# dyfcalid/CameraCalibration

Measured on AMD Instinct MI355X. Metric: stitched BEV frames/sec (4-cam 1280x960->1080x1080), higher is better.
Workload: dtype u8

## Files before the change

cameracalibration_amd/csrc/bevw_unit.h:

```cpp
#pragma once
#include <algorithm>
#include <cstring>
#include <vector>

#ifndef BEVW_UNIT_STORE16
#define BEVW_UNIT_STORE16 0
#endif

namespace bevw {

constexpr int kUnitWaves = 4;
constexpr int kUnitThreads = kUnitWaves * 64;
constexpr int kUnitMaxNQ = 4;
constexpr int kUnitMaxGR = 4;
constexpr int kUnitMaxGroups = kUnitMaxGR * kUnitThreads;
constexpr int kUnitMaxWidth = 256;
constexpr int kUnitClasses = 8;
constexpr int kUnitClassNQ[kUnitClasses] = {4, 4, 2, 1, 2, 1, 1, 4};
constexpr int kUnitClassGR[kUnitClasses] = {1, 2, 4, 4, 1, 4, 1, 4};
constexpr int kUnitClassCON[kUnitClasses] = {1, 1, 1, 1, 2, 2, 2, 1};
constexpr int kUnitClassBig = 7;
constexpr uint32_t kUnitSkip = 1u << 22;

struct UnitDesc {
// ... 19 lines not shown
    return k | (slot0 << 2) | (slot1 << 12) | ((code & 1023u) << 22);
}
__host__ __device__ __forceinline__ void unit_decode(uint32_t e, uint32_t &i0, uint32_t &i1, uint32_t &wxa, uint32_t &wy)
{
    const uint32_t fx = (e >> 22) & 31u, fy = e >> 27;
    i0 = e & 0xfffu;
    i1 = ((e >> 10) & 0xffcu) | (e & 3u);
    wxa = (i0 >> 2) != (i1 >> 2) ? ((32u - fx) | (fx << 8)) : 0u;
    wy = ((32u - fy) << 6) | (fy << 22);
}

constexpr uint32_t kUnitFracBits = 21;
__host__ __device__ __forceinline__ void unit_decode_wide(uint32_t e, uint32_t f, uint32_t &i0, uint32_t &i1, float &fx, float &fy)
{
    i0 = e & 0xfffu;
    i1 = ((e >> 10) & 0xffcu) | (e & 3u);
    fx = (float)((((e >> 22) & 31u) << 16) | (f & 0xffffu)) * (1.0f / (float)(1u << kUnitFracBits));
    fy = (float)(((e >> 27) << 16) | (f >> 16)) * (1.0f / (float)(1u << kUnitFracBits));
}
__host__ __device__ __forceinline__ void unit_repack16(int q, const uint32_t d[3], const uint32_t n[3], uint32_t o[4])
{
    o[0] = q == 0 ? d[0] : (q == 1 ? d[1] : d[2]);
    o[1] = q == 0 ? d[1] : (q == 1 ? d[2] : n[0]);
    o[2] = q == 0 ? d[2] : (q == 1 ? n[0] : n[1]);
    o[3] = q == 0 ? n[0] : (q == 1 ? n[1] : n[2]);
}
__host__ __device__ __forceinline__ bool unit_no_contributor(uint32_t e) { return ((e >> 2) & 1023u) == ((e >> 12) & 1023u); }
__host__ __device__ __forceinline__ uint32_t bilinear_pairs_f32(uint2 q0, uint2 q1, float fx, float fy)
{
    auto lerp = [](float a, float b, float t) { return fmaf(t, b - a, a); };
    auto ch = [&](uint32_t w0, uint32_t w1, int s) {
        const float t = lerp((float)((w0 >> s) & 255u), (float)((w0 >> (s + 8)) & 255u), fx);
        const float b = lerp((float)((w1 >> s) & 255u), (float)((w1 >> (s + 8)) & 255u), fx);
        return (uint32_t)rintf(lerp(t, b, fy));
    };
    return ch(q0.x, q1.x, 0) | (ch(q0.x, q1.x, 16) << 8) | (ch(q0.y, q1.y, 0) << 16);
}

static inline std::vector<uint32_t> unit_host_headers(const std::vector<int16_t> lut1[4], const std::vector<uint8_t> mask[4], int ncams, int fw, int fh,
                                                      int bw, int bh, int tiles_x, int tiles_y);

struct UnitPlanHost {
    std::vector<UnitDesc> desc;
    std::vector<uint32_t> entries;
    std::vector<uint32_t> gsrc;
    std::vector<uint32_t> list[kUnitClasses];
    std::vector<uint32_t> all;
    size_t claimed_tiles = 0;
    uint32_t skew = 0;
    bool wide = false;
    size_t lines = 0, sectors = 0;
    size_t cls_lines[kUnitClasses] = {}, cls_sectors[kUnitClasses] = {}, cls_pixels[kUnitClasses] = {}, cls_groups[kUnitClasses] = {};
};

struct UnitTuning {
    int max_groups = kUnitMaxGroups;
    int root_w = 256, root_h = 64;
    int min_w = 16;
    int line_cost = 2, sector_cost = 3;
    int align_lines = 1;
    int own_empty = 1;
    int own_double = 1;
    int wide_double = 1;
    int skew = 0;
    int row_order = 0;
    int own_padding = 1;
    int run_cost = 0;
    int stagger = 0;
    int big_class = 1;
};

static inline void unit_compile(const std::vector<int16_t> lut1[4], const std::vector<uint16_t> lut2[4], const std::vector<uint8_t> mask[4],
                                int ncams, int fw, int fh, int bw, int bh, int pitch, int tiles_x, int tiles_y, std::vector<uint32_t> &hdr,
                                UnitPlanHost &out, const UnitTuning &tune = UnitTuning(), const std::vector<uint32_t> *frac = nullptr)
{
    const bool wide = frac != nullptr;
    out.wide = wide;
    const uint32_t frame_bytes = (uint32_t)fw * fh * 3, gpr = (uint32_t)fw / 4;
    const size_t set_bytes = (size_t)frame_bytes * ncams;
    constexpr uint32_t kNone = 0xffffffffu;
    std::vector<uint8_t> own((size_t)tiles_x * tiles_y, 0);
    for (size_t t = 0; t < own.size(); ++t) {
        own[t] = (hdr[t] & (kHdrSlow | kHdrBlock)) ? 0 : ((hdr[t] & kHdrSecond) ? (tune.own_double ? 2 : 0) : 1);
        if ((hdr[t] & kHdrEmpty) && !tune.own_empty) own[t] = 0;
    }
    std::vector<uint32_t> poff[2], pcode[2], pfrac[2];
    std::vector<uint8_t> pmask[2];
    for (int k = 0; k < 2; ++k) {
        poff[k].assign((size_t)pitch * bh, kNone); pcode[k].assign((size_t)pitch * bh, 0u); pmask[k].assign((size_t)pitch * bh, 0);
        if (wide) pfrac[k].assign((size_t)pitch * bh, 0u);
    }
    for (int y = 0; y < bh; ++y)
        for (int x = 0; x < bw; ++x) {
            const size_t t = (size_t)(y / 8) * tiles_x + x / 32;
            if (!own[t]) continue;
            const size_t o = (size_t)y * bw + x;
            int count = 0;
            for (int c = 0; c < ncams; ++c) {
                const uint32_t m = mask[c][o];
                if (m == 0) continue;
                const int sx = lut1[c][o * 2], sy = lut1[c][o * 2 + 1];
                if (sx >= fw || sx + 1 < 0 || sy >= fh || sy + 1 < 0) continue;
                const uint32_t off = (uint32_t)c * frame_bytes + ((uint32_t)sy * fw + sx) * 3;
                if ((size_t)(off / 12u + gpr) * 12u + 16u > set_bytes || count >= 2) { own[t] = 0; break; }
                if (m != 255u && own[t] == 1) own[t] = tune.own_double ? 2 : 0;
                poff[count][(size_t)y * pitch + x] = off;
                if (wide) {
                    const uint32_t fx = frac[c][o * 2] & ((1u << kUnitFracBits) - 1u), fy = frac[c][o * 2 + 1] & ((1u << kUnitFracBits) - 1u);
                    pcode[count][(size_t)y * pitch + x] = (fx >> 16) | ((fy >> 16) << 5);
                    pfrac[count][(size_t)y * pitch + x] = (fx & 0xffffu) | (fy << 16);
                } else {
                    pcode[count][(size_t)y * pitch + x] = lut2[c][o] & (kQTab2 - 1);
                }
                pmask[count][(size_t)y * pitch + x] = (uint8_t)m;
                ++count;
            }
        }
    for (int y = 0; y < bh; ++y)
        for (int x = 0; x < bw; ++x)
            if (own[(size_t)(y / 8) * tiles_x + x / 32] == 0) poff[0][(size_t)y * pitch + x] = poff[1][(size_t)y * pitch + x] = kNone;
    int pass = 1;
    const int bw_own = tune.own_padding ? std::min(pitch, tiles_x * 32) : bw;
    auto owned = [&](int x, int y) { return x < bw_own && y < bh && own[(size_t)(y / 8) * tiles_x + x / 32] == pass; };
    const uint32_t P = (uint32_t)pitch * 3u;
    uint32_t skew = 0;
    int col_step = 16;
    if ((tune.skew == 64 || tune.skew == 32) && ((size_t)P * bh) % (size_t)tune.skew == 0) {
        const uint32_t m = (uint32_t)tune.skew / 4u, inv = tune.skew == 64 ? 11u : 3u;
        const uint32_t c = (m - ((P / 4u) * inv) % m) % m;
        if (c != 0) { skew = c | ((m - 1u) << 8); col_step = tune.skew; }
        else col_step = tune.skew;
    }
    out.skew = skew;
    const int min_w = std::max(col_step, tune.min_w);
    auto px_x = [&](int u, int y) { return u + unit_skew(skew, y); };

    std::vector<uint32_t> gstamp(set_bytes / 12 + 2, 0u), lstamp(set_bytes / 128 + 2, 0u);
    uint32_t stamp = 0;
    struct Stats { int groups, lines, pixels, quads; };
    auto cell_stats = [&](int x0, int y0, int w, int h) {
        Stats s = {0, 0, 0, 0};
        ++stamp;
        for (int y = y0; y < y0 + h; ++y)
            for (int u = x0; u < x0 + w; ++u) {
                const int x = px_x(u, y);
                if (x < 0 || x >= pitch) continue;
                if (!owned(x & ~3, y)) continue;
                if ((x & 3) == 0) ++s.quads;
                for (int con = 0; con < 2; ++con) {
                    const uint32_t off = poff[con][(size_t)y * pitch + x];
                    if (off == kNone) continue;
                    ++s.pixels;
                    for (uint32_t r = 0; r < 2; ++r) {
                        const uint32_t k = off / 12u + r * gpr;
                        if (gstamp[k] == stamp) continue;
                        gstamp[k] = stamp;
                        ++s.groups;
                        const uint32_t a = k * 12u;
                        for (uint32_t l = a >> 7; l <= (a + 15u) >> 7; ++l)
                            if (lstamp[l] != stamp) { lstamp[l] = stamp; ++s.lines; }
                    }
                }
            }
        return s;
    };
    auto write_sectors = [&](int x0, int y0, int w, int h) {
        long n = 0;
        for (int y = y0; y < y0 + h; ++y) {
            const int xa = std::max(0, px_x(x0, y)), xb = std::min(pitch, px_x(x0 + w, y));
            int run0 = -1;
            for (int x = xa; x <= xb; x += 4) {
                const bool in = x < xb && owned(x, y);
                if (in && run0 < 0) run0 = x;
                if (!in && run0 >= 0) {
                    const long a0 = ((long)y * pitch + run0) * 3, a1 = ((long)y * pitch + x) * 3;
                    n += (a1 - 1) / 64 - a0 / 64 + 1;
                    run0 = -1;
                }
            }
        }
        return n;
    };
    auto shrink = [&](int &x0, int &y0, int &w, int &h) {
        int ya = y0 + h, yb = y0, ua = x0 + w, ub = x0;
        for (int y = y0; y < y0 + h; ++y)
            for (int u = x0; u < x0 + w; u += 4) {
                const int x = px_x(u, y);
                if (x < 0 || x >= pitch || !owned(x, y)) continue;
                ya = std::min(ya, y); yb = std::max(yb, y + 1); ua = std::min(ua, u); ub = std::max(ub, u + 4);
            }
        if (yb <= ya) return;
        const int xa = x0 + (ua - x0) / col_step * col_step, xb = std::min(x0 + w, x0 + (ub - x0 + col_step - 1) / col_step * col_step);
        x0 = xa; w = xb - xa; y0 = ya; h = yb - ya;
    };
    auto lanes_log2 = [](int w) { int lq = 2; while ((4 << lq) < w) ++lq; return lq; };
    auto slots_needed = [&](int w, int h) { const int rps = 64 >> lanes_log2(w); return (h + rps - 1) / rps; };

    const int root_w = std::min(tune.root_w, kUnitMaxWidth);
    struct Order { uint64_t key; uint32_t entry; uint32_t row; uint64_t cost; };
    auto row_start = [&](int y0) {
        int xs = skew ? -col_step : 0;
        if (tune.stagger > 0) xs -= (((y0 / tune.root_h) * tune.stagger) % root_w) / col_step * col_step;
        return xs;
    };
    std::vector<Order> order;
    std::vector<uint32_t> keys, slot;
    auto emit = [&](int x0, int y0, int w, int h, const Stats &st) {
        keys.clear();
        for (int y = y0; y < y0 + h; ++y)
            for (int u = x0; u < x0 + w; ++u) {
                const int x = px_x(u, y);
                if (x < 0 || x >= pitch || !owned(x & ~3, y)) continue;
                for (int con = 0; con < 2; ++con) {
                    const uint32_t off = poff[con][(size_t)y * pitch + x];
                    if (off == kNone) continue;
                    keys.push_back(off / 12u);
                    keys.push_back(off / 12u + gpr);
                }
            }
        std::sort(keys.begin(), keys.end());
        keys.erase(std::unique(keys.begin(), keys.end()), keys.end());
        const int count = (int)keys.size();
        slot.assign((size_t)count, 0u);
        uint32_t used = 0;
        for (int i = 0; i < count;) {
            int j = i;
            while (j < count && (keys[(size_t)j] * 12u) >> 7 == (keys[(size_t)i] * 12u) >> 7) ++j;
            if (tune.align_lines && (used & 63u) + (uint32_t)(j - i) > 64u) used = (used + 63u) & ~63u;
            for (; i < j; ++i) slot[(size_t)i] = used++;
        }
        const int lq = lanes_log2(w), slots = slots_needed(w, h);
        int cls = -1, best = 1 << 30;
        for (int c = 0; c < kUnitClasses; ++c) {
            if (kUnitClassCON[c] != pass || kUnitClassNQ[c] * kUnitWaves < slots || kUnitClassGR[c] * kUnitThreads < (int)used + (wide ? 1 : 0)) continue;
            if (c == 4 && !tune.wide_double) continue;
            if (c == kUnitClassBig && !tune.big_class) continue;
            const int cost = kUnitClassNQ[c] * 64 + kUnitClassGR[c] * 14;
            if (cost < best) { best = cost; cls = c; }
        }
        if (cls < 0) return false;
        const int NQ = kUnitClassNQ[cls], GR = kUnitClassGR[cls], fpart = pass == 2 ? 3 : 1, parts = fpart + (wide ? pass : 0);
        const uint32_t zent = wide ? unit_entry(used, used, 0u, 0u) : 0u;
        UnitDesc d;
        d.pos = (uint32_t)(uint16_t)(int16_t)x0 | ((uint32_t)y0 << 16);
        d.shape = (uint32_t)w | ((uint32_t)h << 16);
        d.ent_off = (uint32_t)(out.entries.size() / 256);
        d.gs_off = (uint32_t)(out.gsrc.size() / kUnitThreads);
        d.lq = (uint32_t)lq;
        d.sum_tile = 0;
        d.groups = (uint32_t)count;
        d.pixels = (uint32_t)st.pixels;
        auto slot_of = [&](uint32_t key) { return slot[(size_t)(std::lower_bound(keys.begin(), keys.end(), key) - keys.begin())]; };
        const size_t e0 = out.entries.size();
        out.entries.resize(e0 + (size_t)NQ * kUnitWaves * parts * 64 * 4, 0u);
        bool have_sum_tile = false;
        for (int sidx = 0; sidx < NQ * kUnitWaves; ++sidx)
            for (int lane = 0; lane < 64; ++lane) {
                int qx, row;
                unit_quad((uint32_t)lq, sidx, lane, qx, row);
                const int y = y0 + row, x = px_x(x0 + 4 * qx, y);
                uint32_t *e = out.entries.data() + e0 + (((size_t)sidx * parts) * 64 + lane) * 4;
                if (wide)
                    for (int p = 0; p < 4; ++p)
                        for (int con = 0; con < pass; ++con) e[con * 256 + p] = zent;
                if (4 * qx >= w || row >= h || x < 0 || x >= pitch) continue;
                if (!owned(x, y)) { e[0] = zent | kUnitSkip; continue; }
                if (!have_sum_tile) { d.sum_tile = (uint32_t)((y / 8) * tiles_x + x / 32); have_sum_tile = true; }
                for (int p = 0; p < 4; ++p)
                    for (int con = 0; con < pass; ++con) {
                        const uint32_t off = poff[con][(size_t)y * pitch + x + p];
                        if (off == kNone) continue;
                        const uint32_t key = off / 12u, pk = (off - key * 12u) / 3u;
                        e[con * 256 + p] = unit_entry(slot_of(key), slot_of(key + gpr), pk, pcode[con][(size_t)y * pitch + x + p]);
                        if (pass == 2) e[2 * 256 + p] |= (uint32_t)pmask[con][(size_t)y * pitch + x + p] << (8 * con);
                        if (wide) e[(fpart + con) * 256 + p] = pfrac[con][(size_t)y * pitch + x + p];
                    }
            }
        const size_t g0 = out.gsrc.size();
        out.gsrc.resize(g0 + (size_t)GR * kUnitThreads, kPairNoGroup);
        for (int i = 0; i < count; ++i) out.gsrc[g0 + slot[(size_t)i]] = keys[(size_t)i] * 12u;
        out.list[cls].push_back((uint32_t)out.desc.size());
        const size_t ws = (size_t)write_sectors(x0, y0, w, h);
        order.push_back({((uint64_t)(y0 / tune.root_h) << 48) | ((uint64_t)((x0 - row_start(y0)) / root_w) << 32) | (uint64_t)order.size(),
                         (uint32_t)out.desc.size() | ((uint32_t)cls << 28), (uint32_t)(y0 / tune.root_h),
                         (uint64_t)tune.line_cost * (uint64_t)st.lines + (uint64_t)ws});
        out.desc.push_back(d);
        out.lines += (size_t)st.lines;
        out.sectors += ws;
        out.cls_lines[cls] += (size_t)st.lines; out.cls_sectors[cls] += ws; out.cls_pixels[cls] += (size_t)st.pixels; out.cls_groups[cls] += (size_t)count;
        return true;
    };

    struct Cell { int x0, y0, w, h; };
    std::vector<Cell> stack;
    for (pass = 1; pass <= 2; ++pass) {
    for (int y0 = 0; y0 < bh; y0 += tune.root_h)
        for (int x0 = row_start(y0); x0 < pitch; x0 += root_w) stack.push_back({x0, y0, std::min(root_w, pitch - x0), std::min(tune.root_h, bh - y0)});
    std::reverse(stack.begin(), stack.end());
    while (!stack.empty()) {
        Cell c = stack.back();
        stack.pop_back();
        shrink(c.x0, c.y0, c.w, c.h);
        const Stats st = cell_stats(c.x0, c.y0, c.w, c.h);
        if (st.quads == 0) continue;
        bool fits = false;
// ... 207 lines not shown
                            const uint32_t wm = NCON == 2 ? blend_weight_q23((e[2 * 256 + p] >> (8 * con)) & 255u) : 0u;
                            for (int k = 0; k < 3; ++k) {
                                const int v = (int)((acc[k] >> 16) & 255u), c = (blend && NCON == 2) ? (int)blend_apply_q23((uint32_t)v, wm) : v;
                                px[k] = con == 0 ? c : (px[k] + c < 255 ? px[k] + c : 255);
                            }
                        }
                        P[p] = (uint32_t)px[0] | ((uint32_t)px[1] << 8) | ((uint32_t)px[2] << 16);
                        if (sums)
                            for (int k = 0; k < 3; ++k) sums[k] += (uint32_t)px[k];
                    }
                const int x = ux + 4 * qx + unit_skew(up.skew, uy + row);
                st[lane] = !(4 * qx >= uw || row >= uh || x < 0 || x >= pitch || (unit_no_contributor(e[0]) && (e[0] & kUnitSkip)));
                so[lane] = ((size_t)(uy + row) * pitch + x) * 3;
                if (st[lane] && car) {
                    uint32_t c[3];
                    memcpy(c, car + so[lane], 12);
                    add_car(P, c[0], c[1], c[2]);
                }
                pack_pixels(P, od[lane][0], od[lane][1], od[lane][2]);
                nv12_quad(P, yq[lane], uvq[lane]);
                qy[lane] = uy + row;
                qxp[lane] = x;
            }
            if (nv12) {
                for (int lane = 0; lane < 64; ++lane) {
                    if (!st[lane]) continue;
                    const uint32_t yo = nv12_y_offset(pitch, qxp[lane], qy[lane]);
                    memcpy(nv12->img + yo, &yq[lane], 4);
                    for (int k = 0; k < 4; ++k) ++(*nv12->y_written)[yo + k];
                    if (qy[lane] & 1) continue;
                    const uint32_t co = nv12_uv_offset(pitch, nv12->bh, qxp[lane], qy[lane]);
                    memcpy(nv12->img + co, &uvq[lane], 4);
                    for (int k = 0; k < 2; ++k) ++(*nv12->uv_written)[(size_t)(qy[lane] / 2) * (pitch / 2) + qxp[lane] / 2 + k];
                }
                continue;
            }
            for (int lane = 0; lane < 64; ++lane) {
                const int q = lane & 3, l0 = lane & ~3;
                const bool whole = store16 && st[l0] && st[l0 + 1] && st[l0 + 2] && st[l0 + 3];
                if (whole) {
                    if (q == 3) continue;
                    uint32_t o[4];
                    unit_repack16(q, od[lane], od[lane + 1], o);
                    memcpy(out_img + so[lane] + 4 * q, o, 16);
                    if (written) for (int k = 0; k < 16; ++k) ++(*written)[(so[lane] + 4 * q + k) / 3];
                } else if (st[lane]) {
                    memcpy(out_img + so[lane], od[lane], 12);
                    if (written) for (int k = 0; k < 12; ++k) ++(*written)[(so[lane] + k) / 3];
                }
            }
        }
}

#ifndef BEVW_UNIT_DEPTH
#define BEVW_UNIT_DEPTH 2
#endif
#ifndef BEVW_UNIT_NO_BIG
#define BEVW_UNIT_NO_BIG 0
#endif
#ifdef BEVW_EXPERIMENT
#include "bevw_unit_experiments.h"
#endif
__device__ __forceinline__ uint32_t wave_sum_dpp(uint32_t v)
{
    v += (uint32_t)__builtin_amdgcn_update_dpp(0, (int)v, 0xB1, 0xf, 0xf, true);
    v += (uint32_t)__builtin_amdgcn_update_dpp(0, (int)v, 0x4E, 0xf, 0xf, true);
    v += (uint32_t)__builtin_amdgcn_update_dpp(0, (int)v, 0x141, 0xf, 0xf, true);
    v += (uint32_t)__builtin_amdgcn_update_dpp(0, (int)v, 0x140, 0xf, 0xf, true);
    v += (uint32_t)__builtin_amdgcn_update_dpp(0, (int)v, 0x142, 0xa, 0xf, false);
    v += (uint32_t)__builtin_amdgcn_update_dpp(0, (int)v, 0x143, 0xc, 0xf, false);
    return (uint32_t)__builtin_amdgcn_readlane((int)v, 63);
}

__device__ __forceinline__ uint4 unit_plan_load(const uint4 *p)
{
    if (!BEVW_PLAN_NT) return *p;
    const pair_u32x4 v = __builtin_nontemporal_load(reinterpret_cast<const pair_u32x4 *>(p));
    return make_uint4(v.x, v.y, v.z, v.w);
}
__device__ __forceinline__ void unit_store_quad(pair_u32x3 v, __amdgpu_buffer_rsrc_t ro, int off, bool streaming)
{
    if (streaming) __builtin_amdgcn_raw_buffer_store_b96(v, ro, off, 0, kPairStreamAux);
    else __builtin_amdgcn_raw_buffer_store_b96(v, ro, off, 0, kPairStoreAux);
}
__device__ __forceinline__ void unit_store_quad16(uint32_t d0, uint32_t d1, uint32_t d2, __amdgpu_buffer_rsrc_t ro, int off16, int q, bool streaming)
{
    const uint32_t d[3] = {d0, d1, d2};
    const uint32_t n[3] = {(uint32_t)__builtin_amdgcn_update_dpp(0, (int)d0, 0xF9, 0xf, 0xf, false),
                           (uint32_t)__builtin_amdgcn_update_dpp(0, (int)d1, 0xF9, 0xf, 0xf, false),
                           (uint32_t)__builtin_amdgcn_update_dpp(0, (int)d2, 0xF9, 0xf, 0xf, false)};
    uint32_t o[4];
    unit_repack16(q, d, n, o);
    const pair_u32x4 v = {o[0], o[1], o[2], o[3]};
    if (streaming) __builtin_amdgcn_raw_buffer_store_b128(v, ro, off16, 0, kPairStreamAux);
    else __builtin_amdgcn_raw_buffer_store_b128(v, ro, off16, 0, kPairStoreAux);
}
__device__ __forceinline__ void unit_store_dword(uint32_t v, __amdgpu_buffer_rsrc_t ro, int off, bool streaming)
{
    if (streaming) __builtin_amdgcn_raw_buffer_store_b32(v, ro, off, 0, kPairStreamAux);
    else __builtin_amdgcn_raw_buffer_store_b32(v, ro, off, 0, kPairStoreAux);
}
template <bool BLEND, bool SUMS, int NQ, int GR, int NCON, bool WIDE = false, bool NV12 = false, bool OUT_NV12 = false, bool SURF = false>
__device__ __forceinline__ void plan_unit_run(const PlanArgs &a, uint32_t chunk, uint32_t unit, uint8_t *lds, uint4 *wave_sums = nullptr)
{
    static_assert(!SURF || NV12, "surfaces are NV12");
    static_assert(NQ >= 1 && NQ <= kUnitMaxNQ && GR >= 1 && GR <= kUnitMaxGR && (NCON == 1 || NCON == 2), "unit class");
// ... 162 lines not shown
    auto issue = [&](int b, int ring) {
        if constexpr (SURF) {
            __amdgpu_buffer_rsrc_t ry, rc;
#pragma unroll
            for (int r = 0; r < GR; ++r) {
                const uint32_t split = (split_bits >> (8 * r)) & 255u;
                if (split > 0u) {
                    surf_rsrc(0, ry, rc);
                    if ((uint32_t)lane < split) {
                        const pair_u32x2 yv = __builtin_amdgcn_raw_buffer_load_b64(ry, (int)gs[r], 0, kPairLoadAux);
                        const pair_u32x2 cv = __builtin_amdgcn_raw_buffer_load_b64(rc, (int)gc[r], 0, kPairLoadAux);
                        pf[ring][r] = pair_u32x4{yv.x, yv.y, cv.x, cv.y};
                    }
                }
                if (split < 64u) {
                    surf_rsrc(1, ry, rc);
                    if ((uint32_t)lane >= split) {
                        const pair_u32x2 yv = __builtin_amdgcn_raw_buffer_load_b64(ry, (int)gs[r], 0, kPairLoadAux);
                        const pair_u32x2 cv = __builtin_amdgcn_raw_buffer_load_b64(rc, (int)gc[r], 0, kPairLoadAux);
                        pf[ring][r] = pair_u32x4{yv.x, yv.y, cv.x, cv.y};
                    }
                }
            }
            return;
        }
        const uint8_t *src = a.frames + (size_t)frame_of(b) * set_bytes;
        const __amdgpu_buffer_rsrc_t rs = __builtin_amdgcn_make_buffer_rsrc(const_cast<uint8_t *>(src), 0, (uint32_t)set_bytes, kBufferWord3);
#pragma unroll
        for (int r = 0; r < GR; ++r) {
            if (NV12) {
                const pair_u32x2 yv = __builtin_amdgcn_raw_buffer_load_b64(rs, (int)gs[r], 0, kPairLoadAux);
                const pair_u32x2 cv = __builtin_amdgcn_raw_buffer_load_b64(rs, (int)gc[r], 0, kPairLoadAux);
                pf[ring][r] = pair_u32x4{yv.x, yv.y, cv.x, cv.y};
            } else {
                pf[ring][r] = __builtin_amdgcn_raw_buffer_load_b128(rs, (int)gs[r], 0, kPairLoadAux);
            }
        }
    };
    auto land = [&](int ring) {
#pragma unroll
        for (int r = 0; r < GR; ++r) {
            uint4 A, B;
            if (NV12) pair_convert_nv12(pf[ring][r].x, pf[ring][r].y, pf[ring][r].z, pf[ring][r].w, gs[r] != kPairNoGroup, A, B);
            else pair_convert(pf[ring][r].x, pf[ring][r].y, pf[ring][r].z, pf[ring][r].w, A, B);
            uint4 *sp = reinterpret_cast<uint4 *>(lds + (DB ? (ring & 1) * kPatch : 0)) + (r * kUnitThreads + (int)threadIdx.x) * 2;
            sp[0] = A;
            sp[1] = B;
        }
    };
    auto acc_to_px = [](const uint32_t acc[3]) {
        return __builtin_amdgcn_perm(acc[2], __builtin_amdgcn_perm(acc[1], acc[0], 0x0c0c0602u), 0x0c060100u);
    };
#ifdef BEVW_EXPERIMENT_FRAME
    auto frame = [&](int b, int ring) { BEVW_EXPERIMENT_FRAME(b, ring) };
#else
    auto frame = [&](int b, int ring) {
        if (!DB) {
            land(ring);
            block_lds_barrier();
        }
        const uint2 *const pw = reinterpret_cast<const uint2 *>(lds + (DB ? (ring & 1) * kPatch : 0));
        issue(b + D, ring);
        uint32_t d[NQ][3];
        uint32_t tb = 0, tg = 0, tr = 0;
#pragma unroll
        for (int j = 0; j < NQ; ++j) {
            if (WIDE) {
                uint32_t P[4];
#pragma unroll
                for (int p = 0; p < 4; ++p) {
                    uint32_t v = bilinear_pairs_f32(pw[i0[j][0][p]], pw[i1[j][0][p]], __uint_as_float(wxa[j][0][p]), __uint_as_float(wy[j][0][p]));
                    if (NCON == 2) {
                        const uint32_t v1 = bilinear_pairs_f32(pw[i0[j][NCON - 1][p]], pw[i1[j][NCON - 1][p]], __uint_as_float(wxa[j][NCON - 1][p]),
                                                               __uint_as_float(wy[j][NCON - 1][p]));
                        uint32_t px = 0;
#pragma unroll
                        for (int k = 0; k < 3; ++k) {
                            const uint32_t a0 = (v >> (8 * k)) & 255u, a1 = (v1 >> (8 * k)) & 255u;
                            const uint32_t c0 = kWeights ? blend_apply_q23(a0, wq[j][0][p]) : a0, c1 = kWeights ? blend_apply_q23(a1, wq[j][NCON - 1][p]) : a1;
                            px |= min(255u, c0 + c1) << (8 * k);
                        }
                        v = px;
                    }
                    P[p] = v;
                }
                if (car_any) {
                    const pair_u32x3 c = __builtin_amdgcn_raw_buffer_load_b96(rcar, car_off(j), 0, 0);
                    add_car(P, c.x, c.y, c.z);
                }
                pack_pixels(P, d[j][0], d[j][1], d[j][2]);
                continue;
            }
            uint32_t acc[4][3];
#pragma unroll
            for (int p = 0; p < 4; ++p) bilinear_pairs(pw[i0[j][0][p]], pw[i1[j][0][p]], wxa[j][0][p], wxa[j][0][p] << 16, wy[j][0][p], acc[p]);
            if (NCON == 1 && !car_any && !OUT_NV12) {
                pack_accs(acc, d[j][0], d[j][1], d[j][2]);
            } else {
                uint32_t P[4];
                if (NCON == 1) {
#pragma unroll
                    for (int p = 0; p < 4; ++p) P[p] = acc_to_px(acc[p]);
                } else {
#pragma unroll
                    for (int p = 0; p < 4; ++p) {
                        uint32_t acc1[3];
                        bilinear_pairs(pw[i0[j][NCON - 1][p]], pw[i1[j][NCON - 1][p]], wxa[j][NCON - 1][p], wxa[j][NCON - 1][p] << 16, wy[j][NCON - 1][p], acc1);
                        uint32_t px = 0;
#pragma unroll
                        for (int k = 0; k < 3; ++k) {
                            const uint32_t v0 = (acc[p][k] >> 16) & 255u, v1 = (acc1[k] >> 16) & 255u;
                            const uint32_t c0 = kWeights ? blend_apply_q23(v0, wq[j][0][p]) : v0, c1 = kWeights ? blend_apply_q23(v1, wq[j][NCON - 1][p]) : v1;
                            px |= min(255u, c0 + c1) << (8 * k);
                        }
                        P[p] = px;
                    }
                }
                if (car_any) {
                    const pair_u32x3 c = __builtin_amdgcn_raw_buffer_load_b96(rcar, car_off(j), 0, 0);
                    add_car(P, c.x, c.y, c.z);
                }
                if (OUT_NV12) nv12_quad(P, d[j][0], d[j][1]);
                else pack_pixels(P, d[j][0], d[j][1], d[j][2]);
            }
            if (SUMS) {
                tb = __builtin_amdgcn_udot4(d[j][2], 0x00000100u, __builtin_amdgcn_udot4(d[j][1], 0x00010000u, __builtin_amdgcn_udot4(d[j][0], 0x01000001u, tb, false), false), false);
                tg = __builtin_amdgcn_udot4(d[j][2], 0x00010000u, __builtin_amdgcn_udot4(d[j][1], 0x01000001u, __builtin_amdgcn_udot4(d[j][0], 0x00000100u, tg, false), false), false);
                tr = __builtin_amdgcn_udot4(d[j][2], 0x01000001u, __builtin_amdgcn_udot4(d[j][1], 0x00000100u, __builtin_amdgcn_udot4(d[j][0], 0x00010000u, tr, false), false), false);
            }
        }
        if (SUMS) {
            const uint32_t wb = wave_sum_dpp(tb), wg = wave_sum_dpp(tg), wr = wave_sum_dpp(tr);
            if (lane == 0) wave_sums[(ring & 1) * kUnitWaves + wave] = make_uint4(wb, wg, wr, 0u);
        }
        if (DB) land((ring + 1) % D);
        {
            uint8_t *img = a.out + (size_t)frame_of(b) * out_bytes;
            const __amdgpu_buffer_rsrc_t ro = __builtin_amdgcn_make_buffer_rsrc(img, 0, (uint32_t)out_bytes, kBufferWord3);
#pragma unroll
            for (int j = 0; j < NQ; ++j) {
                if (OUT_NV12) store_nv12(j, d[j][0], d[j][1], ro);
                else store_slot(j, d[j][0], d[j][1], d[j][2], ro);
            }
        }
        if constexpr (SURF) surf_fetch(b + D + 1);
        block_lds_barrier();
        if (SUMS && wave == 0 && lane < 3 && b < b_end) {
            const uint32_t *ws = reinterpret_cast<const uint32_t *>(wave_sums + (ring & 1) * kUnitWaves) + lane;
            a.psums[((size_t)b * a.nsum + unit) * 3 + lane] = ws[0] + ws[4] + ws[8] + ws[12];
        }
    };
#endif
#pragma unroll
    for (int u = 0; u < D; ++u) {
        if constexpr (SURF) surf_fetch(b_begin + u);
        issue(b_begin + u, u);
    }
    if constexpr (SURF) surf_fetch(b_begin + D);
#ifndef BEVW_EXPERIMENT_FRAME
    if (DB) {
        land(0);
        block_lds_barrier();
    }
#endif
#pragma unroll 1
    for (int b = b_begin; b < b_end; b += D) {
#pragma unroll
        for (int u = 0; u < D; ++u) frame(b + u, u);
    }
}

template <bool BLEND, bool SUMS, bool NV12, bool OUT_NV12 = false, bool SURF = false>
__device__ __forceinline__ void plan_unit_any(const PlanArgs &a, uint32_t block_id, uint8_t *lds, uint4 *wave_sums)
{
    uint32_t chunk, group;
    if (!plan_block_map(a, block_id, chunk, group)) return;
    if ((int)group >= a.nlist) return;
    const uint32_t e = __builtin_amdgcn_readfirstlane(a.tile_list[group]), unit = e & 0x0fffffffu;
#define BEVW_UNIT_CASE(C) case C: plan_unit_run<BLEND, SUMS, kUnitClassNQ[C], kUnitClassGR[C], kUnitClassCON[C], false, NV12, OUT_NV12, SURF>(a, chunk, unit, lds, wave_sums); break;
    switch (e >> 28) {
        BEVW_UNIT_CASE(0) BEVW_UNIT_CASE(1) BEVW_UNIT_CASE(2) BEVW_UNIT_CASE(3)
        BEVW_UNIT_CASE(4)
        BEVW_UNIT_CASE(5)
#if !BEVW_UNIT_NO_BIG
        BEVW_UNIT_CASE(7)
#endif
        default: plan_unit_run<BLEND, SUMS, kUnitClassNQ[6], kUnitClassGR[6], kUnitClassCON[6], false, NV12, OUT_NV12, SURF>(a, chunk, unit, lds, wave_sums); break;
    }
#undef BEVW_UNIT_CASE
}

#ifndef BEVW_PLAN_ALL_WAVES
#define BEVW_PLAN_ALL_WAVES 3
#endif
template <bool BLEND, bool SUMS>
__global__ void __launch_bounds__(kUnitThreads) __attribute__((amdgpu_waves_per_eu(BEVW_PLAN_ALL_WAVES, BEVW_PLAN_ALL_WAVES))) k_plan_units(PlanArgs a)
{
    __shared__ __attribute__((aligned(16))) uint8_t patch[kUnitMaxGroups * 32];
    __shared__ uint4 wave_sums[SUMS ? 2 * kUnitWaves : 1];
#ifdef BEVW_EXPERIMENT_TRACE_BEGIN
    BEVW_EXPERIMENT_TRACE_BEGIN();
#endif
    plan_unit_any<BLEND, SUMS, false>(a, blockIdx.x, patch, wave_sums);
#ifdef BEVW_EXPERIMENT_TRACE_END
    BEVW_EXPERIMENT_TRACE_END(a)
#endif
}

template <bool BLEND>
__global__ void __launch_bounds__(kUnitThreads) __attribute__((amdgpu_waves_per_eu(BEVW_PLAN_ALL_WAVES, BEVW_PLAN_ALL_WAVES))) k_units_nv12(PlanArgs a)
{
    __shared__ __attribute__((aligned(16))) uint8_t patch[kUnitMaxGroups * 32];
    plan_unit_any<BLEND, false, true>(a, blockIdx.x, patch, nullptr);
}

template <bool BLEND, bool IN_NV12>
__global__ void __launch_bounds__(kUnitThreads) __attribute__((amdgpu_waves_per_eu(BEVW_PLAN_ALL_WAVES, BEVW_PLAN_ALL_WAVES))) k_units_out_nv12(PlanArgs a)
{
    __shared__ __attribute__((aligned(16))) uint8_t patch[kUnitMaxGroups * 32];
    plan_unit_any<BLEND, false, IN_NV12, true>(a, blockIdx.x, patch, nullptr);
}
// ... 33 lines not shown
```

cameracalibration_amd/csrc/bevwarp_plan.hip:

```cpp
#include "bevw_plan.h"

namespace bevw {

void plan_release(Plan &p)
{
    void *ptrs[] = {p.un_desc, p.un_entries, p.un_gsrc, p.un_gsrc_compact, p.un_gsrc_nv12, p.list_un_all, p.entries, p.hdr, p.groups, p.groups_nv12, p.un_gsrc_surf, p.groups_surf, p.psums, p.pad_out, p.pad_car, p.d_max, p.list_slow};
    for (void *q : ptrs)
        if (q) (void)hipFree(q);
    p = Plan();
}

const uint32_t *plan_sum_entries(const Plan &p, int first, int &nsum)
{
    nsum = p.psums_layout;
    return static_cast<const uint32_t *>(p.psums) + (size_t)first * (size_t)(nsum > 0 ? nsum : 0) * 3;
}

static UnitTuning unit_tuning_env()
{
    UnitTuning t;
    if (const char *s = getenv("BEVW_UNIT_GROUPS")) t.max_groups = atoi(s);
    if (const char *s = getenv("BEVW_UNIT_ROOT_W")) t.root_w = atoi(s);
    if (const char *s = getenv("BEVW_UNIT_ROOT_H")) t.root_h = atoi(s);
    if (const char *s = getenv("BEVW_UNIT_MIN_W")) t.min_w = atoi(s);
    if (const char *s = getenv("BEVW_UNIT_LINE_COST")) t.line_cost = atoi(s);
    if (const char *s = getenv("BEVW_UNIT_SECTOR_COST")) t.sector_cost = atoi(s);
    if (const char *s = getenv("BEVW_UNIT_ALIGN_LINES")) t.align_lines = atoi(s);
    if (const char *s = getenv("BEVW_UNIT_OWN_EMPTY")) t.own_empty = atoi(s);
    if (const char *s = getenv("BEVW_UNIT_SKEW")) t.skew = atoi(s);
    if (const char *s = getenv("BEVW_UNIT_ROW_ORDER")) t.row_order = atoi(s);
    if (const char *s = getenv("BEVW_UNIT_OWN_PADDING")) t.own_padding = atoi(s);
    if (const char *s = getenv("BEVW_UNIT_STAGGER")) t.stagger = atoi(s);
    if (const char *s = getenv("BEVW_UNIT_RUN_COST")) t.run_cost = atoi(s);
    if (const char *s = getenv("BEVW_UNIT_BIG")) t.big_class = atoi(s);
    if (const char *s = getenv("BEVW_UNIT_WIDE_DOUBLE")) t.wide_double = atoi(s);
    return t;
}

static const PlanTuning &plan_tuning()
{
    static const PlanTuning tune = [] {
        PlanTuning t;
        if (const char *s = getenv("BEVW_PLAN_NB")) t.nb = atoi(s);
        if (const char *s = getenv("BEVW_PLAN_XCDMAP")) t.xcd_map = atoi(s);
        if (const char *s = getenv("BEVW_PLAN_UNITS")) t.units = atoi(s);
        return t;
    }();
    return tune;
}

int plan_build(Plan &p, hipStream_t st, const StitchTables &T, int fw, int fh, int bw, int bh, int ncams, int out_pitch, bool blend)
{
    static const UnitTuning unit_tune = unit_tuning_env();
    UnitTuning tune = unit_tune;
    (void)blend;
    if (out_pitch > 0 && !getenv("BEVW_UNIT_SECTOR_COST")) tune.sector_cost = 8;
    if (ncams == 1 && !getenv("BEVW_UNIT_ROW_ORDER")) tune.row_order = 4;
    hipError_t e = plan_build_impl(p, st, T, fw, fh, bw, bh, ncams, plan_tuning().units != 0, tune, out_pitch);
    if (e != hipSuccess) return fail(BEVW_E_HIP, "tile-plan build failed: %s", hipGetErrorString(e));
    return BEVW_OK;
}

int plan_stitch(Plan &p, hipStream_t st, const uint8_t *d_frames, int batch, bool blend, bool balance, const int *d_deltas, const HsvTables *d_tab,
                const uint8_t *d_car, unsigned long long *d_chsums, uint8_t *d_out, bool sums, int psums_frames, int psums_first, const uint8_t *d_scratch,
                const Nv12Surface *d_surf)
{
    hipError_t e = plan_stitch_impl(p, st, d_frames, batch, blend, balance, d_deltas, d_tab, d_car, d_chsums, d_out, plan_tuning(), sums, psums_frames,
                                    psums_first, d_scratch, d_surf);
    if (e != hipSuccess) return fail(BEVW_E_HIP, "tile-plan stitch launch failed: %s", hipGetErrorString(e));
    return BEVW_OK;
}

int plan_set_src_pitch(Plan &p, int pitch)
{
    hipError_t e = plan_src_pitch_impl(p, pitch);
    if (e != hipSuccess) return fail(BEVW_E_HIP, "uploading the surface group lists failed: %s", hipGetErrorString(e));
    return BEVW_OK;
}

int plan_lum_groups(const Plan &p, hipStream_t st, const uint8_t *d_frames, uint8_t *d_scratch, int batch, const int *d_deltas, const HsvTables *d_tab,
                    const Nv12Surface *d_surf)
{
    hipError_t e = plan_lum_band(p, st, d_frames, d_scratch, batch, d_deltas, d_tab, d_surf);
    if (e != hipSuccess) return fail(BEVW_E_HIP, "k_lum_groups launch failed: %s", hipGetErrorString(e));
    return BEVW_OK;
}

int plan_pad_image(hipStream_t st, const uint8_t *d_src, int bw, int pitch, int bh, uint8_t *d_dst)
// ... 52 lines not shown
```

Measured before the change: 641,200.

## Assign LDS group slots to minimize bank conflicts and trim pipeline tail work

The unit compiler now simulates, per lane half-wave, which LDS banks each gathered group hits. It chooses slot offsets (up to 8 pads per cache-line cluster) that reduce the modeled conflict cost, and falls back to plain packing if that is no better or overflows capacity. The kernel loop is also split into a steady phase and a tail phase, so it stops issuing loads, landings and surface fetches past the batch end. The output frame index no longer goes through frame_of. This adds host-side plan compile cost, and the unused-slot padding may raise LDS footprint.

```diff
diff --git a/cameracalibration_amd/csrc/bevw_unit.h b/cameracalibration_amd/csrc/bevw_unit.h
--- a/cameracalibration_amd/csrc/bevw_unit.h
+++ b/cameracalibration_amd/csrc/bevw_unit.h
@@ -95,6 +95,14 @@
     size_t lines = 0, sectors = 0;
     size_t cls_lines[kUnitClasses] = {}, cls_sectors[kUnitClasses] = {}, cls_pixels[kUnitClasses] = {}, cls_groups[kUnitClasses] = {};
 };
+
+__host__ __device__ __forceinline__ uint32_t unit_lds_bank(uint32_t q) { return q & 31u; }
+#ifdef BEVW_HOST_EMULATOR
+static bool g_unit_plain_dealing = false;
+static inline bool unit_plain_dealing() { return g_unit_plain_dealing; }
+#else
+constexpr bool unit_plain_dealing() { return false; }
+#endif
 
 struct UnitTuning {
     int max_groups = kUnitMaxGroups;
@@ -111,6 +119,7 @@
     int run_cost = 0;
     int stagger = 0;
     int big_class = 1;
+    int bank_deal = 1;
 };
 
 static inline void unit_compile(const std::vector<int16_t> lut1[4], const std::vector<uint16_t> lut2[4], const std::vector<uint8_t> mask[4],
@@ -178,7 +187,7 @@
     const int min_w = std::max(col_step, tune.min_w);
     auto px_x = [&](int u, int y) { return u + unit_skew(skew, y); };
 
-    std::vector<uint32_t> gstamp(set_bytes / 12 + 2, 0u), lstamp(set_bytes / 128 + 2, 0u);
+    std::vector<uint32_t> gstamp(set_bytes / 12 + 2, 0u), lstamp(set_bytes / 128 + 2, 0u), kmap(set_bytes / 12 + 2, 0u);
     uint32_t stamp = 0;
     struct Stats { int groups, lines, pixels, quads; };
     auto cell_stats = [&](int x0, int y0, int w, int h) {
@@ -247,7 +256,8 @@
         return xs;
     };
     std::vector<Order> order;
-    std::vector<uint32_t> keys, slot;
+    std::vector<uint32_t> keys, slot, cl_first, cl_plain, acc_stamp, acc_n, acc_tmp, acc_list, acc_fill, bank_try, bank_add;
+    std::vector<uint8_t> zero_h, bank_cnt, bank_max;
     auto emit = [&](int x0, int y0, int w, int h, const Stats &st) {
         keys.clear();
         for (int y = y0; y < y0 + h; ++y)
@@ -264,14 +274,18 @@
         std::sort(keys.begin(), keys.end());
         keys.erase(std::unique(keys.begin(), keys.end()), keys.end());
         const int count = (int)keys.size();
+        for (int i = 0; i < count; ++i) kmap[keys[(size_t)i]] = (uint32_t)i;
         slot.assign((size_t)count, 0u);
+        cl_first.clear(); cl_plain.clear();
         uint32_t used = 0;
         for (int i = 0; i < count;) {
             int j = i;
             while (j < count && (keys[(size_t)j] * 12u) >> 7 == (keys[(size_t)i] * 12u) >> 7) ++j;
             if (tune.align_lines && (used & 63u) + (uint32_t)(j - i) > 64u) used = (used + 63u) & ~63u;
+            cl_first.push_back((uint32_t)i); cl_plain.push_back(used);
             for (; i < j; ++i) slot[(size_t)i] = used++;
         }
+        cl_first.push_back((uint32_t)count);
         const int lq = lanes_log2(w), slots = slots_needed(w, h);
         int cls = -1, best = 1 << 30;
         for (int c = 0; c < kUnitClasses; ++c) {
@@ -283,6 +297,102 @@
         }
         if (cls < 0) return false;
         const int NQ = kUnitClassNQ[cls], GR = kUnitClassGR[cls], fpart = pass == 2 ? 3 : 1, parts = fpart + (wide ? pass : 0);
+        if (tune.bank_deal && !unit_plain_dealing() && count > 0) {
+            const int nslot = NQ * kUnitWaves, nh = nslot * pass * 4 * 2 * 2;
+            const uint32_t cap = (uint32_t)(GR * kUnitThreads) - (wide ? 1u : 0u);
+            acc_stamp.assign((size_t)count * 8, 0u);
+            acc_n.assign((size_t)count + 1, 0u);
+            acc_tmp.clear();
+            zero_h.assign((size_t)nh, 0);
+            for (int sidx = 0; sidx < nslot; ++sidx)
+                for (int con = 0; con < pass; ++con)
+                    for (int p = 0; p < 4; ++p)
+                        for (int lane = 0; lane < 64; ++lane) {
+                            int qx, row;
+                            unit_quad((uint32_t)lq, sidx, lane, qx, row);
+                            const int y = y0 + row, x = px_x(x0 + 4 * qx, y);
+                            const uint32_t hid = (uint32_t)((((sidx * pass + con) * 4 + p) * 2) * 2 + (lane >> 5));
+                            uint32_t off = kNone;
+                            if (!(4 * qx >= w || row >= h || x < 0 || x >= pitch) && owned(x, y)) off = poff[con][(size_t)y * pitch + x + p];
+                            if (off == kNone) { zero_h[hid] = zero_h[hid + 2] = 1; continue; }
+                            const uint32_t key = off / 12u, pk = (off - key * 12u) / 3u;
+                            for (uint32_t r = 0; r < 2; ++r) {
+                                const uint32_t ki = kmap[key + r * gpr];
+                                const uint32_t h = hid + 2u * r;
+                                uint32_t &seen = acc_stamp[((size_t)ki * 4 + pk) * 2 + r];
+                                if (seen == h + 1u) continue;
+                                seen = h + 1u;
+                                acc_tmp.push_back((ki << 12) | (h << 2) | pk);
+                                ++acc_n[ki + 1];
+                            }
+                        }
+            for (int i = 0; i < count; ++i) acc_n[(size_t)i + 1] += acc_n[(size_t)i];
+            acc_list.resize(acc_tmp.size());
+            acc_fill.assign(acc_n.begin(), acc_n.end() - 1);
+            for (uint32_t a : acc_tmp) acc_list[acc_fill[a >> 12]++] = a & 0xfffu;
+            bank_try.assign((size_t)nh, 0u);
+            auto reset = [&]() {
+                bank_cnt.assign((size_t)nh * 32, 0);
+                bank_max.assign((size_t)nh, 0);
+                if (!wide)
+                    for (int hh = 0; hh < nh; ++hh)
+                        if (zero_h[(size_t)hh]) { bank_cnt[(size_t)hh * 32] = 1; bank_max[(size_t)hh] = 1; }
+            };
+            uint32_t try_id = 0;
+            bank_add.assign((size_t)nh * 32, 0u);
+            auto place = [&](uint32_t gi, uint32_t gj, uint32_t S, bool commit) {
+                uint32_t cost = 0;
+                ++try_id;
+                for (uint32_t g = gi; g < gj; ++g) {
+                    const uint32_t sl = S + (g - gi);
+                    for (uint32_t q = acc_n[g]; q < acc_n[(size_t)g + 1]; ++q) {
+                        const uint32_t h = acc_list[q] >> 2, k = acc_list[q] & 3u;
+                        if (sl == 0 && k == 0 && !wide && zero_h[h]) continue;
+                        const size_t at = (size_t)h * 32 + unit_lds_bank(4u * sl + k);
+                        uint32_t c;
+                        if (commit) {
+                            c = ++bank_cnt[at];
+                        } else {
+                            const uint32_t add = (bank_add[at] >> 8) == try_id ? (bank_add[at] & 255u) + 1u : 1u;
+                            bank_add[at] = (try_id << 8) | add;
+                            c = bank_cnt[at] + add;
+                        }
+                        const uint32_t m = (bank_try[h] >> 8) == try_id ? (bank_try[h] & 255u) : bank_max[h];
+                        if (c > m) { cost += c - m; bank_try[h] = (try_id << 8) | c; if (commit) bank_max[h] = (uint8_t)c; }
+                    }
+                }
+                return cost;
+            };
+            const uint32_t ncl = (uint32_t)cl_plain.size();
+            uint32_t plain_cost = 0, deal_cost = 0;
+            reset();
+            for (uint32_t c = 0; c < ncl; ++c) plain_cost += place(cl_first[c], cl_first[(size_t)c + 1], cl_plain[c], true);
+            reset();
+            used = 0;
+            for (uint32_t c = 0; c < ncl; ++c) {
+                const uint32_t gi = cl_first[c], gj = cl_first[(size_t)c + 1], n = gj - gi;
+                uint32_t best_s = 0, best_cost = 0xffffffffu, last_s = 0xffffffffu;
+                for (uint32_t pad = 0; pad < 8; ++pad) {
+                    uint32_t S = used + pad;
+                    if (tune.align_lines && (S & 63u) + n > 64u) S = ((used + 63u) & ~63u) + pad;
+                    if (S == last_s) continue;
+                    last_s = S;
+                    const uint32_t rest = (uint32_t)count - gi, bounds = (cap - 1u) / 64u - std::min(S, cap - 1u) / 64u;
+                    if (S != cl_plain[c] && (S + rest + (tune.align_lines ? 10u * bounds : 0u) > cap || (S & 63u) + n > 64u)) continue;
+                    const uint32_t cost = place(gi, gj, S, false);
+                    if (cost < best_cost) { best_cost = cost; best_s = S; }
+                }
+                if (best_cost == 0xffffffffu) best_s = (tune.align_lines && (used & 63u) + n > 64u) ? ((used + 63u) & ~63u) : used;
+                deal_cost += place(gi, gj, best_s, true);
+                for (uint32_t g = gi; g < gj; ++g) slot[g] = best_s + (g - gi);
+                used = best_s + n;
+            }
+            if (used > cap || deal_cost >= plain_cost) {
+                used = 0;
+                for (uint32_t c = 0; c < ncl; ++c)
+                    for (uint32_t g = cl_first[c]; g < cl_first[(size_t)c + 1]; ++g) { slot[g] = cl_plain[c] + (g - cl_first[c]); used = slot[g] + 1; }
+            }
+        }
         const uint32_t zent = wide ? unit_entry(used, used, 0u, 0u) : 0u;
         UnitDesc d;
         d.pos = (uint32_t)(uint16_t)(int16_t)x0 | ((uint32_t)y0 << 16);
@@ -293,7 +403,7 @@
         d.sum_tile = 0;
         d.groups = (uint32_t)count;
         d.pixels = (uint32_t)st.pixels;
-        auto slot_of = [&](uint32_t key) { return slot[(size_t)(std::lower_bound(keys.begin(), keys.end(), key) - keys.begin())]; };
+        auto slot_of = [&](uint32_t key) { return slot[kmap[key]]; };
         const size_t e0 = out.entries.size();
         out.entries.resize(e0 + (size_t)NQ * kUnitWaves * parts * 64 * 4, 0u);
         bool have_sum_tile = false;
@@ -607,6 +717,35 @@
         }
 }
 
+struct UnitChunkSchedule { int issues = 0, frames = 0, lands = 0; bool ok = true; };
+static inline UnitChunkSchedule unit_chunk_schedule(int n, int D, bool DB)
+{
+    UnitChunkSchedule s;
+    std::vector<int> ring((size_t)D, -1), done((size_t)std::max(n, 0), 0);
+    int half[2] = {-1, -1};
+    auto issue = [&](int b, int r) { ring[(size_t)r] = b; ++s.issues; s.ok = s.ok && b < n; };
+    auto land = [&](int r) { half[DB ? (r & 1) : 0] = ring[(size_t)r]; ++s.lands; s.ok = s.ok && ring[(size_t)r] >= 0; };
+    auto frame = [&](int b, int r, bool steady) {
+        if (!DB) land(r);
+        s.ok = s.ok && half[DB ? (r & 1) : 0] == b;
+        if (steady || b + D < n) issue(b + D, r);
+        if (DB && (steady || b + 1 < n)) land((r + 1) % D);
+        ++s.frames;
+        if (b < n) ++done[(size_t)b]; else s.ok = false;
+    };
+    for (int u = 0; u < D; ++u)
+        if (u < n) issue(u, u);
+    if (DB && n > 0) land(0);
+    int b = 0;
+    for (; b + 2 * D <= n; b += D)
+        for (int u = 0; u < D; ++u) frame(b + u, u, true);
+    for (; b < n; b += D)
+        for (int u = 0; u < D; ++u)
+            if (b + u < n) frame(b + u, u, false);
+    for (int d : done) s.ok = s.ok && d == 1;
+    return s;
+}
+
 #ifndef BEVW_UNIT_DEPTH
 #define BEVW_UNIT_DEPTH 2
 #endif
@@ -875,15 +1014,15 @@
         return __builtin_amdgcn_perm(acc[2], __builtin_amdgcn_perm(acc[1], acc[0], 0x0c0c0602u), 0x0c060100u);
     };
 #ifdef BEVW_EXPERIMENT_FRAME
-    auto frame = [&](int b, int ring) { BEVW_EXPERIMENT_FRAME(b, ring) };
+    auto frame = [&](int b, int ring, bool) { BEVW_EXPERIMENT_FRAME(b, ring) };
 #else
-    auto frame = [&](int b, int ring) {
+    auto frame = [&](int b, int ring, bool steady) {
         if (!DB) {
             land(ring);
             block_lds_barrier();
         }
         const uint2 *const pw = reinterpret_cast<const uint2 *>(lds + (DB ? (ring & 1) * kPatch : 0));
-        issue(b + D, ring);
+        if (steady || b + D < b_end) issue(b + D, ring);
         uint32_t d[NQ][3];
         uint32_t tb = 0, tg = 0, tr = 0;
 #pragma unroll
@@ -956,9 +1095,9 @@
             const uint32_t wb = wave_sum_dpp(tb), wg = wave_sum_dpp(tg), wr = wave_sum_dpp(tr);
             if (lane == 0) wave_sums[(ring & 1) * kUnitWaves + wave] = make_uint4(wb, wg, wr, 0u);
         }
-        if (DB) land((ring + 1) % D);
+        if (DB && (steady || b + 1 < b_end)) land((ring + 1) % D);
         {
-            uint8_t *img = a.out + (size_t)frame_of(b) * out_bytes;
+            uint8_t *img = a.out + (size_t)b * out_bytes;
             const __amdgpu_buffer_rsrc_t ro = __builtin_amdgcn_make_buffer_rsrc(img, 0, (uint32_t)out_bytes, kBufferWord3);
 #pragma unroll
             for (int j = 0; j < NQ; ++j) {
@@ -966,7 +1105,9 @@
                 else store_slot(j, d[j][0], d[j][1], d[j][2], ro);
             }
         }
-        if constexpr (SURF) surf_fetch(b + D + 1);
+        if constexpr (SURF) {
+            if (steady || b + D + 1 < b_end) surf_fetch(b + D + 1);
+        }
         block_lds_barrier();
         if (SUMS && wave == 0 && lane < 3 && b < b_end) {
             const uint32_t *ws = reinterpret_cast<const uint32_t *>(wave_sums + (ring & 1) * kUnitWaves) + lane;
@@ -976,8 +1117,10 @@
 #endif
 #pragma unroll
     for (int u = 0; u < D; ++u) {
-        if constexpr (SURF) surf_fetch(b_begin + u);
-        issue(b_begin + u, u);
+        if (b_begin + u < b_end) {
+            if constexpr (SURF) surf_fetch(b_begin + u);
+            issue(b_begin + u, u);
+        }
     }
     if constexpr (SURF) surf_fetch(b_begin + D);
 #ifndef BEVW_EXPERIMENT_FRAME
@@ -986,10 +1129,17 @@
         block_lds_barrier();
     }
 #endif
+    int b = b_begin;
 #pragma unroll 1
-    for (int b = b_begin; b < b_end; b += D) {
-#pragma unroll
-        for (int u = 0; u < D; ++u) frame(b + u, u);
+    for (; b + 2 * D <= b_end; b += D) {
+#pragma unroll
+        for (int u = 0; u < D; ++u) frame(b + u, u, true);
+    }
+#pragma unroll 1
+    for (; b < b_end; b += D) {
+#pragma unroll
+        for (int u = 0; u < D; ++u)
+            if (b + u < b_end) frame(b + u, u, false);
     }
 }
 
diff --git a/cameracalibration_amd/csrc/bevwarp_plan.hip b/cameracalibration_amd/csrc/bevwarp_plan.hip
--- a/cameracalibration_amd/csrc/bevwarp_plan.hip
+++ b/cameracalibration_amd/csrc/bevwarp_plan.hip
@@ -34,6 +34,7 @@
     if (const char *s = getenv("BEVW_UNIT_RUN_COST")) t.run_cost = atoi(s);
     if (const char *s = getenv("BEVW_UNIT_BIG")) t.big_class = atoi(s);
     if (const char *s = getenv("BEVW_UNIT_WIDE_DOUBLE")) t.wide_double = atoi(s);
+    if (const char *s = getenv("BEVW_UNIT_BANK_DEAL")) t.bank_deal = atoi(s);
     return t;
 }
 
```

New measurement: 645,200 (median of 6 runs). Within noise of the previous version (+0.6%).
